# penn-pal-lab/robot_aware_control

Measured on AMD Instinct MI355X. Metric: SVG train frames/sec + CEM candidate-rollouts/sec, 64x64, higher is better.
Workload: dtype fp32 (conv operands as two fp16 parts = 22 significant bits, fp32 accumulate; see fp32_exact)

## Files before the change

### robot_aware_control_amd/csrc/rac_split16.hip

```cpp
#include <math.h>
#include <stdlib.h>

#include <type_traits>

#include "rac_common.h"

namespace rac {

typedef _Float16 f16x8 __attribute__((ext_vector_type(8)));
typedef _Float16 f16x4 __attribute__((ext_vector_type(4)));
typedef unsigned int u32x4 __attribute__((ext_vector_type(4)));
typedef unsigned int u32x2 __attribute__((ext_vector_type(2)));
typedef __amdgpu_buffer_rsrc_t rsrc_t;

constexpr unsigned OOB = 0xFFFFFFF0u;
constexpr int SBN = 128, SBK = 32;

__device__ __forceinline__ const void* uniform_ptr(const void* p) {
  unsigned long long v = reinterpret_cast<unsigned long long>(p);
  unsigned lo = __builtin_amdgcn_readfirstlane((unsigned)v);
  unsigned hi = __builtin_amdgcn_readfirstlane((unsigned)(v >> 32));
  return reinterpret_cast<const void*>(((unsigned long long)hi << 32) | lo);
}
__device__ __forceinline__ rsrc_t make_rsrc(const void* p, unsigned bytes) {
// ... 1560 lines not shown
#pragma unroll
          for (int t = 0; t < HB; ++t) read_frag(t, (tap + 1) % 9, cur * abuf);
        }
        __builtin_amdgcn_sched_barrier(0);
#pragma unroll
        for (int t = HB; t < MB; ++t)
#pragma unroll
          for (int nb = 0; nb < NB; ++nb) acc[t][nb] = mma3(fa[t], fb[nb], acc[t][nb]);
      }
    }
    const int img = p.per_image ? cur_t.m0 / p.HW : 0;
    if (RAC_EXP_PERSIST & 2) {
      unsigned mx = 0;
#pragma unroll
      for (int i = 0; i < MB; ++i)
#pragma unroll
        for (int j = 0; j < NB; ++j)
#pragma unroll
          for (int r = 0; r < 4; ++r) mx = max(mx, absbits(acc[i][j][r]));
      if (p.out_amax) amax_commit(mx, p.out_amax + img);
    } else {
      conv16_epilogue(p, acc, cur_t.m0, wm * MB, nmb, n0 + wn * NT * 32, 0, pow2f(-cur_t.ka), pow2f(-kw), pre, nullptr,
                      p.out_amax ? p.out_amax + img : nullptr);
    }
    if (!has_next) break;
    cur ^= 1;
    cur_t = nxt_t;
    bx = next_bx;
  }
}

__global__ __launch_bounds__(256) void absmax_kernel(const float4* x0, long n0v, const float4* x1, long n1v,
                                                     unsigned* amax) {
  __shared__ unsigned sh[4];
  unsigned m = 0;
  const long stride = (long)gridDim.x * blockDim.x;
  for (long i = (long)blockIdx.x * blockDim.x + threadIdx.x; i < n0v + n1v; i += stride) {
    const float4 v = i < n0v ? x0[i] : x1[i - n0v];
    const unsigned a = __builtin_bit_cast(unsigned, v.x) & 0x7FFFFFFFu, b = __builtin_bit_cast(unsigned, v.y) & 0x7FFFFFFFu,
                   c = __builtin_bit_cast(unsigned, v.z) & 0x7FFFFFFFu, d = __builtin_bit_cast(unsigned, v.w) & 0x7FFFFFFFu;
    m = max(m, max(max(a, b), max(c, d)));
  }
#pragma unroll
  for (int o = 32; o > 0; o >>= 1) m = max(m, (unsigned)__shfl_xor((int)m, o));
  if ((threadIdx.x & 63) == 0) sh[threadIdx.x >> 6] = m;
  __syncthreads();
  if (threadIdx.x == 0) {
    m = max(max(sh[0], sh[1]), max(sh[2], sh[3]));
    if (m > __hip_atomic_load(amax, __ATOMIC_RELAXED, __HIP_MEMORY_SCOPE_AGENT)) atomicMax(amax, m);
  }
}

__device__ __forceinline__ void weight_frag16_block(const float* w, const unsigned* w_amax, unsigned short* out, int Cout,
                                                    int Cin, int taps, int transposed, long ps, long block) {
  const int R = transposed ? Cin : Cout, Kc = transposed ? Cout : Cin;
  const int cch = Kc >> 5;
  const long cell = block * 2 + (threadIdx.x >> 7);
  if (cell >= (long)(R >> 5) * cch * taps) return;
  const float s = pow2f(scale_exp(*w_amax));
  const int tap = (int)(cell % taps);
  const int cc = (int)((cell / taps) % cch);
  const int nt = (int)(cell / ((long)taps * cch));
  const int nb = (threadIdx.x >> 6) & 1, lane = threadIdx.x & 63;
  const int r = nt * 32 + nb * 16 + (lane & 15);
  const int k0 = cc * 32 + 8 * (lane >> 4);
  u32x4 lo, hi;
  if (!transposed) {
    const u32x4* src = reinterpret_cast<const u32x4*>(w + ((long)r * taps + tap) * Cin + k0);
    lo = src[0], hi = src[1];
  } else {
    unsigned v[8];
#pragma unroll
    for (int j = 0; j < 8; ++j)
      v[j] = __builtin_bit_cast(unsigned, w[((long)(k0 + j) * taps + (taps - 1 - tap)) * Cin + r]);
    lo = u32x4{v[0], v[1], v[2], v[3]}, hi = u32x4{v[4], v[5], v[6], v[7]};
  }
  u32x4 q[2];
  split8h(lo, hi, s, q);
  const long o = (cell * 2 + nb) * 512 + lane * 8;
  *reinterpret_cast<u32x4*>(out + o) = q[0];
  *reinterpret_cast<u32x4*>(out + ps + o) = q[1];
}

__global__ void weight_frag16_kernel(const float* w, const unsigned* w_amax, unsigned short* out, int Cout, int Cin,
                                     int taps, int transposed, long ps) {
  weight_frag16_block(w, w_amax, out, Cout, Cin, taps, transposed, ps, blockIdx.x);
}

template <typename Job>
__device__ __forceinline__ int job_of_block(const Job* jobs, int n_jobs, long block) {
  int lo = 0, hi = n_jobs - 1;
  while (lo < hi) {
    const int mid = (lo + hi + 1) >> 1;
    if (jobs[mid].block_begin <= block) lo = mid; else hi = mid - 1;
  }
  return lo;
}

__global__ void weight_frag16_multi_kernel(const rac_frag_job* jobs, int n_jobs) {
  const int j = job_of_block(jobs, n_jobs, blockIdx.x);
  const rac_frag_job q = jobs[j];
  weight_frag16_block(q.w, q.w_amax, q.parts, q.Cout, q.Cin, q.ksize * q.ksize, q.transposed, q.part_stride,
                      blockIdx.x - q.block_begin);
}

__global__ __launch_bounds__(256) void absmax_multi_kernel(const rac_absmax_job* jobs, int n_jobs) {
  __shared__ unsigned sh[4];
  const int j = job_of_block(jobs, n_jobs, blockIdx.x);
  const rac_absmax_job q = jobs[j];
  const long nb = (j + 1 < n_jobs ? jobs[j + 1].block_begin : (long)gridDim.x) - q.block_begin;
  const float4* x = reinterpret_cast<const float4*>(q.x);
  const long nv = q.n >> 2;
  unsigned m = 0;
  for (long i = (blockIdx.x - q.block_begin) * 256 + threadIdx.x; i < nv; i += nb * 256) {
    const float4 v = x[i];
    m = max(m, max(max(absbits(v.x), absbits(v.y)), max(absbits(v.z), absbits(v.w))));
  }
#pragma unroll
  for (int o = 32; o > 0; o >>= 1) m = max(m, (unsigned)__shfl_xor((int)m, o));
  if ((threadIdx.x & 63) == 0) sh[threadIdx.x >> 6] = m;
  __syncthreads();
  if (threadIdx.x == 0) {
    m = max(max(sh[0], sh[1]), max(sh[2], sh[3]));
    if (m > __hip_atomic_load(q.amax, __ATOMIC_RELAXED, __HIP_MEMORY_SCOPE_AGENT)) atomicMax(q.amax, m);
  }
}


__global__ __launch_bounds__(256) void adam_frag_multi_kernel(const rac_adam_frag_job* jobs, int n_jobs, long total_blocks,
                                                              float b1, float b2, float eps, float step_size,
                                                              float inv_sqrt_bc2) {
  __shared__ float tile[2][32][33];
  __shared__ unsigned mx_sh[4];
  for (long blk = blockIdx.x; blk < total_blocks; blk += gridDim.x) {
  const int j = job_of_block(jobs, n_jobs, (int)blk);
  const rac_adam_frag_job q = jobs[j];
  const int taps = q.ksize * q.ksize, cch = q.Cin >> 5;
  const int half = threadIdx.x >> 7;
  const long cell = (blk - q.block_begin) * 2 + half;
  const bool active = cell < (long)(q.Cout >> 5) * cch * taps;
  const int tap = (int)(cell % taps);
  const int cc = (int)((cell / taps) % cch);
  const int nt = (int)(cell / ((long)taps * cch));
  const int nb = (threadIdx.x >> 6) & 1, lane = threadIdx.x & 63;
  const int rl = nb * 16 + (lane & 15), kl = 8 * (lane >> 4);
  const float s = pow2f(scale_exp(*q.scale_slot));
  unsigned mx = 0;
  if (active) {
    const long off = ((long)(nt * 32 + rl) * taps + tap) * q.Cin + cc * 32 + kl;
    f32x4 P[2], G[2], M[2], V[2];
#pragma unroll
    for (int h = 0; h < 2; ++h) {
      P[h] = *reinterpret_cast<const f32x4*>(q.p + off + 4 * h);
      G[h] = *reinterpret_cast<const f32x4*>(q.g + off + 4 * h);
      M[h] = *reinterpret_cast<const f32x4*>(q.m + off + 4 * h);
      V[h] = *reinterpret_cast<const f32x4*>(q.v + off + 4 * h);
#pragma unroll
      for (int e = 0; e < 4; ++e) {
        float pp = P[h][e], mm = M[h][e], vv = V[h][e];
        adam_update(pp, G[h][e], mm, vv, b1, b2, eps, step_size, inv_sqrt_bc2);
        M[h][e] = mm, V[h][e] = vv, P[h][e] = pp;
        mx = max(mx, absbits(pp));
        tile[half][rl][kl + 4 * h + e] = pp;
      }
      *reinterpret_cast<f32x4*>(q.p + off + 4 * h) = P[h];
      *reinterpret_cast<f32x4*>(q.m + off + 4 * h) = M[h];
      *reinterpret_cast<f32x4*>(q.v + off + 4 * h) = V[h];
    }
    if (q.parts_fwd) {
      u32x4 parts[2];
      split8h(__builtin_bit_cast(u32x4, P[0]), __builtin_bit_cast(u32x4, P[1]), s, parts);
      const long o = (cell * 2 + nb) * 512 + lane * 8;
      *reinterpret_cast<u32x4*>(q.parts_fwd + o) = parts[0];
      *reinterpret_cast<u32x4*>(q.parts_fwd + q.part_stride + o) = parts[1];
    }
  }
  __syncthreads();
  if (active && q.parts_t) {
    float v[8];
#pragma unroll
    for (int e = 0; e < 8; ++e) v[e] = tile[half][kl + e][rl];
    u32x4 parts[2];
    split8h(u32x4{__builtin_bit_cast(unsigned, v[0]), __builtin_bit_cast(unsigned, v[1]), __builtin_bit_cast(unsigned, v[2]),
                  __builtin_bit_cast(unsigned, v[3])},
            u32x4{__builtin_bit_cast(unsigned, v[4]), __builtin_bit_cast(unsigned, v[5]), __builtin_bit_cast(unsigned, v[6]),
                  __builtin_bit_cast(unsigned, v[7])}, s, parts);
    const long cell_t = ((long)cc * (q.Cout >> 5) + nt) * taps + (taps - 1 - tap);
    const long o = (cell_t * 2 + nb) * 512 + lane * 8;
    *reinterpret_cast<u32x4*>(q.parts_t + o) = parts[0];
    *reinterpret_cast<u32x4*>(q.parts_t + q.part_stride + o) = parts[1];
  }
#pragma unroll
  for (int o = 32; o > 0; o >>= 1) mx = max(mx, (unsigned)__shfl_xor((int)mx, o));
  if (lane == 0) mx_sh[threadIdx.x >> 6] = mx;
  __syncthreads();
  if (threadIdx.x == 0) {
    mx = max(max(mx_sh[0], mx_sh[1]), max(mx_sh[2], mx_sh[3]));
    if (mx > __hip_atomic_load(q.amax_out, __ATOMIC_RELAXED, __HIP_MEMORY_SCOPE_AGENT)) atomicMax(q.amax_out, mx);
  }
  }
}

__global__ void amax_bound_kernel(unsigned* exact, unsigned* bound, const int* idx, int n, float margin) {
  const int j = blockIdx.x * blockDim.x + threadIdx.x;
  if (j >= n) return;
  const int i = idx[j];
  bound[i] = __builtin_bit_cast(unsigned, __builtin_bit_cast(float, exact[i]) + margin);
  exact[i] = 0;
}


struct Wgrad16P {
  int Bimg, H, W, Cin, Cout, C0, T;
  int R, G;
  int nsplit, accumulate;
  int nseg;
  int x1_skip;
  int presplit;
  const float* dy[RAC_WGRAD_MAX_STEPS];
  const float* x0[RAC_WGRAD_MAX_STEPS];
// ... 566 lines not shown
  u32x4* d0 = reinterpret_cast<u32x4*>(p.parts[t]);
  u32x4* d1 = d0 + p.n8;
  for (long i = (long)blockIdx.x * 256 + threadIdx.x; i < p.n8; i += (long)gridDim.x * 256) {
    u32x4 q[2];
    split8h(src[2 * i], src[2 * i + 1], s, q);
    d0[i] = q[0];
    d1[i] = q[1];
  }
}

__global__ __launch_bounds__(256) void slab_accumulate_many_kernel(const float4* slabs, int n_slabs, long stride4,
                                                                   float4* out, long n4) {
  __shared__ float4 sh[256];
  const int col = threadIdx.x & 15, lane = threadIdx.x >> 4;
  const long i = (long)blockIdx.x * 16 + col;
  float4 a = {0.f, 0.f, 0.f, 0.f};
  if (i < n4)
    for (int s = lane; s < n_slabs; s += 16) {
      const float4 b = slabs[s * stride4 + i];
      a.x += b.x, a.y += b.y, a.z += b.z, a.w += b.w;
    }
  sh[threadIdx.x] = a;
  __syncthreads();
  if (lane == 0 && i < n4) {
    float4 r = out[i];
    for (int k = 0; k < 16; ++k) {
      const float4 b = sh[k * 16 + col];
      r.x += b.x, r.y += b.y, r.z += b.z, r.w += b.w;
    }
    out[i] = r;
  }
}

}

using namespace rac;

extern "C" int rac_absmax(const float* x0, int64_t n0, const float* x1, int64_t n1, uint32_t* amax, void* stream) {
  RAC_REQUIRE(x0 && n0 > 0 && n1 >= 0 && (n1 == 0 || x1) && amax, "rac_absmax: bad args");
  RAC_REQUIRE(n0 % 4 == 0 && n1 % 4 == 0 && aligned16(x0) && (!x1 || aligned16(x1)),
              "rac_absmax: element counts must be multiples of 4, pointers 16-byte aligned");
  long nb = ((n0 + n1) / 4 + 1023) / 1024;
  if (nb > 512) nb = 512;
  hipLaunchKernelGGL(absmax_kernel, dim3((int)nb), dim3(256), 0, reinterpret_cast<hipStream_t>(stream),
                     reinterpret_cast<const float4*>(x0), (long)(n0 / 4), reinterpret_cast<const float4*>(x1),
                     (long)(n1 / 4), amax);
  return check_launch("rac_absmax");
}

extern "C" int rac_weight_frag_split(const float* w, const uint32_t* w_amax, uint16_t* parts, int32_t Cout, int32_t Cin,
                                     int32_t ksize, int32_t transposed, int64_t part_stride, void* stream) {
  RAC_REQUIRE(w && w_amax && parts && Cout > 0 && Cin > 0 && ksize >= 1 && (ksize & 1), "rac_weight_frag_split: bad args");
  RAC_REQUIRE(Cout % 32 == 0 && Cin % 32 == 0, "rac_weight_frag_split: channel counts must be multiples of 32");
  const long n = (long)Cout * Cin * ksize * ksize;
  RAC_REQUIRE(part_stride >= n && part_stride % 8 == 0 && aligned16(w) && aligned16(parts),
              "rac_weight_frag_split: part stride / alignment");
  const long cells = n / 1024;
  hipLaunchKernelGGL(weight_frag16_kernel, dim3((unsigned)((cells + 1) / 2)), dim3(256), 0,
                     reinterpret_cast<hipStream_t>(stream), w, w_amax, parts, Cout, Cin, ksize * ksize, transposed,
                     (long)part_stride);
  return check_launch("rac_weight_frag_split");
}

extern "C" int64_t rac_absmax_blocks(int64_t n) {
  long nb = (n / 4 + 1023) / 1024;
  return nb < 1 ? 1 : (nb > 512 ? 512 : nb);
}

extern "C" int64_t rac_weight_frag_blocks(int32_t Cout, int32_t Cin, int32_t ksize) {
  return ((long)Cout * Cin * ksize * ksize / 1024 + 1) / 2;
}

extern "C" int rac_absmax_multi(const rac_absmax_job* jobs, int32_t n_jobs, int64_t total_blocks, void* stream) {
  RAC_REQUIRE(jobs && n_jobs > 0 && total_blocks >= n_jobs && total_blocks < 0x7FFFFFFFL, "rac_absmax_multi: bad args");
  hipLaunchKernelGGL(absmax_multi_kernel, dim3((unsigned)total_blocks), dim3(256), 0,
                     reinterpret_cast<hipStream_t>(stream), jobs, n_jobs);
  return check_launch("rac_absmax_multi");
}

extern "C" int rac_weight_frag_split_multi(const rac_frag_job* jobs, int32_t n_jobs, int64_t total_blocks, void* stream) {
  RAC_REQUIRE(jobs && n_jobs > 0 && total_blocks >= n_jobs && total_blocks < 0x7FFFFFFFL,
              "rac_weight_frag_split_multi: bad args");
  hipLaunchKernelGGL(weight_frag16_multi_kernel, dim3((unsigned)total_blocks), dim3(256), 0,
                     reinterpret_cast<hipStream_t>(stream), jobs, n_jobs);
  return check_launch("rac_weight_frag_split_multi");
}

extern "C" int rac_adam_frag_multi(const rac_adam_frag_job* jobs, int32_t n_jobs, int64_t total_blocks, float lr, float beta1,
                                   float beta2, float eps, int32_t step, void* stream) {
  RAC_REQUIRE(jobs && n_jobs > 0 && total_blocks >= n_jobs && total_blocks < 0x7FFFFFFFL && step >= 1,
              "rac_adam_frag_multi: bad args");
  const double bc1 = 1.0 - pow((double)beta1, step), bc2 = 1.0 - pow((double)beta2, step);
  hipLaunchKernelGGL(adam_frag_multi_kernel, dim3((unsigned)total_blocks), dim3(256), 0, reinterpret_cast<hipStream_t>(stream),
                     jobs, n_jobs, (long)total_blocks, beta1, beta2, eps, (float)((double)lr / bc1), (float)(1.0 / sqrt(bc2)));
  return check_launch("rac_adam_frag_multi");
}

extern "C" int rac_adam_frag_multi_bounded(const rac_adam_frag_job* jobs, int32_t n_jobs, int64_t total_blocks,
                                           int32_t max_workgroups, float lr, float beta1, float beta2, float eps, int32_t step,
                                           void* stream) {
  RAC_REQUIRE(jobs && n_jobs > 0 && total_blocks > 0 && total_blocks < (1L << 31) && step >= 1 && max_workgroups >= 1,
              "rac_adam_frag_multi_bounded: bad args");
  const double bc1 = 1.0 - pow((double)beta1, step), bc2 = 1.0 - pow((double)beta2, step);
  const long grid = total_blocks < max_workgroups ? total_blocks : max_workgroups;
  hipLaunchKernelGGL(adam_frag_multi_kernel, dim3((unsigned)grid), dim3(256), 0, reinterpret_cast<hipStream_t>(stream), jobs,
                     n_jobs, (long)total_blocks, beta1, beta2, eps, (float)((double)lr / bc1), (float)(1.0 / sqrt(bc2)));
// ... 420 lines not shown
```

### robot_aware_control_amd/ops.py

```python
from __future__ import annotations

import contextlib
import ctypes as C
import functools
import os
import weakref
from typing import Optional, Tuple

import torch

from . import _lib
from ._lib import (AbsmaxJob, AdamFragJob, AdamRange, ConvArgs, FragJob, GradSrc, OptimRange, WgradArgs, call, ptr,
                   stream_ptr)

FWD, DGRAD, WGRAD = 0, 1, 2
ACT_NONE, ACT_LEAKY, ACT_SIGMOID = 0, 1, 2
LOSS_KINDS = {"mse": 0, "l1": 1, "dontcare_mse": 2, "dontcare_l1": 3}
BN_EPS, BN_MOMENTUM = 1e-5, 0.1


def _require_cuda(t: torch.Tensor):
    if not t.is_cuda:
        raise _lib.RacError("robot_aware_control_amd ops run on the GPU only (no CPU fallback); got a CPU tensor")

# ... 2 lines not shown
    co, ci, kh, kw = w.shape
    if w.stride() != (kh * kw * ci, 1, kw * ci, ci):
        raise _lib.RacError(f"conv weight {tuple(w.shape)} must use channels_last memory, strides {w.stride()}")
    return w


_STALE = {}
LAZY_ZERO_GRAD = os.environ.get("RAC_LAZY_ZERO_GRAD", "1") == "1"


def mark_stale(g: torch.Tensor) -> None:
    _STALE[g.data_ptr()] = g


def take_stale(g: torch.Tensor) -> bool:
    return bool(_STALE) and _STALE.pop(g.data_ptr(), None) is not None


def finish_grads() -> None:
    for g in _STALE.values():
        g.zero_()
    _STALE.clear()


def grad_buffer(p: torch.Tensor) -> torch.Tensor:
    if p.grad is None:
        p.grad = torch.zeros_like(p)
    elif _STALE and take_stale(p.grad):
        p.grad.zero_()
    return p.grad


def _cdiv(a, b):
    return (a + b - 1) // b


PARAM_EPOCH = 0


def pad4(c: int) -> int:
    return (-c) % 4


def _derived(weight: torch.Tensor, slot: str, build):
    tag = (weight._version, PARAM_EPOCH, weight.data_ptr())
    hit = getattr(weight, slot, None)
    if hit is not None and hit[0] == tag:
        return hit[1]
    val = build()
    setattr(weight, slot, (tag, val))
    return val


def padded_weight(weight: torch.Tensor, cp: Optional[int] = None) -> torch.Tensor:
    co, ci, k, _ = weight.shape
    cp = ci + pad4(ci) if cp is None else cp

    def build():
        wp = getattr(weight, f"_rac_padbuf{cp}", None)
        if wp is None or wp.device != weight.device:
            wp = torch.empty((co, k, k, cp), device=weight.device, dtype=torch.float32).permute(0, 3, 1, 2)
            setattr(weight, f"_rac_padbuf{cp}", wp)
            wp._rac_pad_source = (weakref.ref(weight), cp)
        call("rac_pad_rows", ptr(weight_mem(weight)), ci, ptr(wp), cp, co * k * k, stream_ptr())
        ent = _WP_ENTRIES.get(id(wp))
        if ent is not None:
            ent.tag = None
        return wp
    return _derived(weight, f"_rac_padded{cp}", build)


def wgrad_padded_acc(dy, x0, weight):
    co, ci, k, _ = weight.shape
    cp = x0.shape[3]
    gp = torch.zeros((co, k, k, cp), device=dy.device, dtype=torch.float32).permute(0, 3, 1, 2)
    B, H, W, Cout = dy.shape
    conv_raw(WGRAD, x0, None, dy, gp, B=B, H=H, W=W, ksize=k, Cin=cp, Cout=Cout, a_split=cp, accumulate=1, split_k=0)
    call("rac_unpad_add", ptr(gp), cp, ptr(weight_mem(grad_buffer(weight))), ci, co * k * k, stream_ptr())


def thin_wgrad_acc(wide, thin, ct: int, weight):
    B, H, W, _ = wide.shape
    n = 64 * 9 * ct
    n_parts = min(512, B * (H // 16) * (W // 16))
    parts = torch.empty((n_parts, n), device=wide.device, dtype=torch.float32)
    sp = stream_ptr()
    call("rac_thin_wgrad", ptr(wide), ptr(thin), thin.shape[3], ct, ptr(parts), n_parts, B, H, W, 64, sp)
    call("rac_slab_accumulate", ptr(parts), n_parts, n, ptr(weight_mem(grad_buffer(weight))), n, sp)


MAX_SPLIT_K = int(os.environ.get("RAC_MAX_SPLIT_K", "8"))


def plan_split_k(M: int, N: int, nchunks: int, tile128_only: bool = False) -> int:
    return _plan_split_k(M, N, nchunks, tile128_only, os.environ.get("RAC_SPLIT"), MAX_SPLIT_K)


@functools.lru_cache(maxsize=None)
def _plan_split_k(M, N, nchunks, tile128_only, forced, max_split):
    if forced:
        return max(1, min(int(forced), nchunks))
    cap = max(1, nchunks // 8)
    if tile128_only:
        t128 = _cdiv(M, 128) * _cdiv(N, 128)
        if t128 >= 384:
            return 1
        best, best_eff = 1, -1.0
        for s in range(1, min(max_split, cap) + 1):
            rounds = t128 * s / 512.0
            eff = (rounds / -(-rounds // 1) if rounds > 1 else rounds) * (1.0 - 0.03 * (s - 1))
            if eff > best_eff + 1e-9:
                best, best_eff = s, eff
        return best
    if N <= 32:
        tiles = _cdiv(M, 128)
        return 1 if tiles >= 384 else max(1, min(8, _cdiv(512, tiles), cap))
    if M >= 128 and N >= 128:
        t128 = _cdiv(M, 128) * _cdiv(N, 128)
        if t128 >= 384:
            return 1
        split = max(1, min(8, _cdiv(512, t128), cap))
        if t128 * split >= 192:
            return split
    tiles = _cdiv(M, 64) * _cdiv(N, 64)
    if tiles >= 384:
        return 1
    return max(1, min(8, _cdiv(512, tiles), cap))


PROFILE = None
SHAPE_LOG = [] if os.environ.get("RAC_SHAPE_LOG") else None
if SHAPE_LOG is not None:
    import atexit
    import json as _json
    atexit.register(lambda: _json.dump(SHAPE_LOG, open(os.environ["RAC_SHAPE_LOG"], "w")))


def _log_shape(family, mode, k, M, N, K, peak):
    SHAPE_LOG.append({"family": family, "mode": ("fwd", "dgrad", "wgrad")[mode], "k": k, "M": M, "N": N, "K": K,
                      "flop": 2.0 * M * N * K, "peak": peak})


def conv_raw(mode: int, a0, a1, w, out0, out1=None, *, B, H, W, ksize, Cin, Cout, act=ACT_NONE, split_k=1,
             slab_stride=0, accumulate=0, a_split=0, o_split=0, bias=None, scale=None, shift=None, stats=None,
             stats_rows=0):
    prof = PROFILE
    if prof is not None and prof["match"] == (mode, ksize, Cin, Cout):
        e0, e1 = torch.cuda.Event(enable_timing=True), torch.cuda.Event(enable_timing=True)
        e0.record()
        _conv_launch(mode, a0, a1, w, out0, out1, B, H, W, ksize, Cin, Cout, act, split_k, slab_stride, accumulate,
                     a_split, o_split, bias, scale, shift, stats, stats_rows)
        e1.record()
        prof["events"].append((e0, e1, B * H * W))
        return
    _conv_launch(mode, a0, a1, w, out0, out1, B, H, W, ksize, Cin, Cout, act, split_k, slab_stride, accumulate,
                 a_split, o_split, bias, scale, shift, stats, stats_rows)


def _conv_launch(mode, a0, a1, w, out0, out1, B, H, W, ksize, Cin, Cout, act, split_k, slab_stride, accumulate,
                 a_split, o_split, bias, scale, shift, stats, stats_rows=0):
    args = ConvArgs(mode=mode, B=B, H=H, W=W, ksize=ksize, Cin=Cin, Cout=Cout, act=act, split_k=split_k,
                    accumulate=accumulate, a_split=a_split, o_split=o_split, slab_stride=slab_stride,
                    a0=ptr(a0), a1=ptr(a1), w=ptr(w), out0=ptr(out0), out1=ptr(out1), bias=ptr(bias),
                    scale=ptr(scale), shift=ptr(shift), stats=ptr(stats), stats_rows=stats_rows)
    if SHAPE_LOG is not None:
        M, N, K = B * H * W, (Cout if mode == FWD else Cin), (Cin if mode == FWD else Cout) * ksize * ksize
        if mode == WGRAD:
            M, N, K = Cout, Cin * ksize * ksize, B * H * W
        _log_shape("igemm", mode, ksize, M, N, K, 157.3)
    call("rac_conv2d", C.byref(args), stream_ptr())


def conv_forward(x0, x1, weight, bias=None, *, act=ACT_NONE, scale=None, shift=None, stats=None,
                 allow_split=True, want_slabs=False, groups=1, frozen=False):
    _require_cuda(x0)
    B, H, W, C0 = x0.shape
    C1 = x1.shape[3] if x1 is not None else 0
    Cout, Cin, k, _ = weight.shape
    assert Cin == C0 + C1, (Cin, C0, C1)
    weight_mem(weight)
    M = B * H * W
    nchunks = k * k * _cdiv(Cin, 32)
    fused = act != ACT_NONE or scale is not None
    split = plan_split_k(M, Cout, nchunks) if (allow_split and not fused and not frozen) else 1
    if want_slabs:
        slabs = torch.empty((split, B, H, W, Cout), device=x0.device, dtype=torch.float32)
        if split == 1:
            conv_raw(FWD, x0, x1, weight, slabs, B=B, H=H, W=W, ksize=k, Cin=Cin, Cout=Cout, a_split=C0)
        else:
            conv_raw(FWD, x0, x1, weight, slabs, B=B, H=H, W=W, ksize=k, Cin=Cin, Cout=Cout, a_split=C0,
                     split_k=split, slab_stride=M * Cout)
        return slabs, split, M * Cout
    out = torch.empty((B, H, W, Cout), device=x0.device, dtype=torch.float32)
    if split == 1:
        conv_raw(FWD, x0, x1, weight, out, B=B, H=H, W=W, ksize=k, Cin=Cin, Cout=Cout, a_split=C0, act=act,
                 bias=bias, scale=scale, shift=shift, stats=stats,
                 stats_rows=(M // groups if (groups > 1 and stats is not None) else 0))
    else:
# ... 135 lines not shown
def broadcast_images(t: torch.Tensor, n: int) -> torch.Tensor:
    out = t.expand(n, *t.shape[1:]).contiguous()
    slot = amax_tag(t)
    if slot is not None:
        if getattr(slot, "_rac_bound1", False):
            tag_amax(out, amax_one(t.device, n))
        elif slot.numel() == 1:
            tag_amax(out, slot.expand(n).contiguous())
    return out


_SPLIT_OK = {}


def split_supported(H: int, W: int, k: int, Cin: int, Cout: int, a_split: int = 0) -> bool:
    key = (H, W, k, Cin, Cout, a_split)
    ok = _SPLIT_OK.get(key)
    if ok is None:
        ok = _SPLIT_OK[key] = bool(_lib.load().rac_conv2d_split_supported(H, W, k, Cin, Cout, a_split))
    return ok


class _WeightParts:
    __slots__ = ("ref", "idx", "slot", "device", "parts", "tag", "exact_ok", "__weakref__")


_WP_ENTRIES = {}
_WP_DEV = {}
_WP_NSLOTS = 1024


def _wp_state(device):
    st = _WP_DEV.get(device)
    if st is None:
        st = _WP_DEV[device] = {"slots": torch.zeros(_WP_NSLOTS, device=device, dtype=torch.int32),
                                "exact": torch.zeros(_WP_NSLOTS, device=device, dtype=torch.int32),
                                "free": list(range(_WP_NSLOTS - 1, -1, -1)), "tables": {}, "adam_plan": None,
                                "optim_plan": None}
    return st


def _wp_drop(key, device, idx, _ref):
    ent = _WP_ENTRIES.get(key)
    if ent is not None and ent.idx == idx and ent.device == device:
        del _WP_ENTRIES[key]
        st = _WP_DEV.get(device)
        if st is not None:
            st["free"].append(idx)


def _wp_tag(weight):
    src = getattr(weight, "_rac_sources", None)
    ver = weight._version if src is None else tuple(t._version for t in src)
    return (ver, PARAM_EPOCH, weight.data_ptr())


def _wp_upload(jobs, device):
    raw = bytes(jobs)
    return torch.frombuffer(bytearray(raw), dtype=torch.uint8).to(device)


ADAM_LATE_WGS = int(os.environ.get("RAC_ADAM_LATE_WGS", "512"))
ADAM_WGS = int(os.environ.get("RAC_ADAM_WGS", "0"))


PARAM_GATE = None


def param_wait(t: torch.Tensor = None) -> None:
    gate = PARAM_GATE
    if gate is None:
        return
    if t is None:
        gate.wait_params()
    elif hasattr(gate, "wait_for"):
        gate.wait_for(t)
    elif not gate.ready(t):
        gate.wait_params()


def _wp_tables(st, items, device):
    lib = _lib.load()
    sig = tuple((w.data_ptr(), ent.idx, tuple(sorted((t, q.data_ptr()) for t, q in ent.parts.items())))
                for ent, w in items)
    tables = st["tables"].get(sig)
    if tables is None:
        if len(st["tables"]) > 8:
            st["tables"].clear()
        ajobs = (AbsmaxJob * len(items))()
        nfrag = sum(len(ent.parts) for ent, _ in items)
        fjobs = (FragJob * nfrag)()
        ab = fb = j = 0
        for i, (ent, w) in enumerate(items):
            wm = weight_mem(w.detach())
            co, ci, k, _ = w.shape
            ajobs[i] = AbsmaxJob(x=ptr(wm), n=wm.numel(), amax=ptr(ent.slot), block_begin=ab)
            ab += lib.rac_absmax_blocks(wm.numel())
            for transposed, parts in sorted(ent.parts.items()):
                fjobs[j] = FragJob(w=ptr(wm), w_amax=ptr(ent.slot), parts=ptr(parts), part_stride=wm.numel(), Cout=co,
                                   Cin=ci, ksize=k, transposed=1 if transposed else 0, block_begin=fb)
                fb += lib.rac_weight_frag_blocks(co, ci, k)
                j += 1
        idx = torch.tensor([ent.idx for ent, _ in items], device=device, dtype=torch.long)
        tables = st["tables"][sig] = (_wp_upload(ajobs, device), len(items), ab, _wp_upload(fjobs, device), nfrag, fb, idx)
    return tables


def _wp_refresh(device):
    st = _wp_state(device)
    stale, n_live = [], 0
    gate = PARAM_GATE
    for ent in list(_WP_ENTRIES.values()):
        if ent.device != device:
            continue
        w = ent.ref()
        if w is None:
            continue
        src = getattr(w, "_rac_pad_source", None)
        if gate is not None:
            base = src[0]() if src is not None else w
            if base is not None and not gate.ready(base):
                continue
        if src is not None:
            param = src[0]()
            if param is None:
                continue
            padded_weight(param, src[1])
        n_live += 1
        if ent.tag != _wp_tag(w):
            stale.append((ent, w))
    if not stale:
        return
    sp = stream_ptr()
    if len(stale) <= 2:
        for ent, w in stale:
            ent.slot.zero_()
            wm = weight_mem(w.detach())
            co, ci, k, _ = w.shape
            call("rac_absmax", ptr(wm), wm.numel(), None, 0, ptr(ent.slot), sp)
            for transposed, parts in ent.parts.items():
                call("rac_weight_frag_split", ptr(wm), ptr(ent.slot), ptr(parts), co, ci, k, 1 if transposed else 0,
                     wm.numel(), sp)
            st["exact"][ent.idx:ent.idx + 1].copy_(ent.slot)
            ent.tag, ent.exact_ok = _wp_tag(w), True
        return
    ta, na, ab, tf, nf, fb, idx = _wp_tables(st, stale, device)
    st["slots"].index_fill_(0, idx, 0)
    call("rac_absmax_multi", ptr(ta), na, ab, sp)
    call("rac_weight_frag_split_multi", ptr(tf), nf, fb, sp)
    st["exact"].index_copy_(0, idx, st["slots"].index_select(0, idx))
    for ent, w in stale:
        ent.tag, ent.exact_ok = _wp_tag(w), True


ADAM_FUSED = os.environ.get("RAC_ADAM_FUSED", "1") == "1"
_ADAM_BOUNDS = {}


def adam_step_bound(beta1: float, beta2: float):
    key = (beta1, beta2)
    if key not in _ADAM_BOUNDS:
        r = beta1 * beta1 / beta2
        if not (0.0 <= beta1 < 1.0 and 0.0 < beta2 < 1.0 and r < 1.0):
            _ADAM_BOUNDS[key] = None
        else:
            best, series, b1t, b2t, rk = 0.0, 0.0, 1.0, 1.0, 1.0
            for _ in range(200000):
                series += rk
                rk *= r
                b1t *= beta1
                b2t *= beta2
                best = max(best, (1 - beta1) ** 2 / (1 - b1t) ** 2 * (1 - b2t) / (1 - beta2) * series)
                if rk < 1e-18 and b1t < 1e-18 and b2t < 1e-9:
                    break
            _ADAM_BOUNDS[key] = best ** 0.5
    return _ADAM_BOUNDS[key]


def _wp_covered(flat):
    dev = flat.device
    base, nbytes = flat.data_ptr(), flat.numel() * 4
    covered = []
    for ent in _WP_ENTRIES.values():
        if ent.device != dev:
            continue
        w = ent.ref()
        if w is None or getattr(w, "_rac_pad_source", None) is not None:
            continue
        off = w.data_ptr() - base
        co, ci, k, _ = w.shape
        if not (0 <= off < nbytes and off % 16 == 0 and w.stride() == (k * k * ci, 1, k * ci, ci)):
            continue
        if ent.tag != _wp_tag(w) or not ent.exact_ok:
            return None
        covered.append((off // 4, ent, w))
    covered.sort(key=lambda c: c[0])
    return covered


def fused_adam_step(flat, grad, m, v, lr, beta1, beta2, eps, step, late=None):
    global PARAM_EPOCH
    if not ADAM_FUSED:
        return False
    bound = adam_step_bound(beta1, beta2)
    if bound is None:
        return False
    dev = flat.device
    st = _wp_state(dev)
    base = flat.data_ptr()
    covered = _wp_covered(flat)
    if not covered:
        return False
    late_sets = [] if late is None else (list(late[1]) if isinstance(late[1], (list, tuple)) else [late[1]])

    def late_group(off, w):
        if late is None or off < late[0]:
            return -1
        for gi, ptrs in enumerate(late_sets):
            if w.data_ptr() in ptrs:
                return gi
        return -1
    is_late = lambda off, w: late_group(off, w) >= 0
    sig = (base, grad.data_ptr(), m.data_ptr(), v.data_ptr(),
           None if late is None else (late[0], tuple(tuple(sorted(ps)) for ps in late_sets)),
           tuple((off, ent.idx, tuple(sorted((t, q.data_ptr()) for t, q in ent.parts.items()))) for off, ent, _ in covered))
    plan = st["adam_plan"]
    if plan is not None and plan["sig"] == sig and plan.get("unsupported"):
        return False
    if plan is None or plan["sig"] != sig:
        lib = _lib.load()
        jobs = (AdamFragJob * len(covered))()
        groups = [late_group(off, w) for off, _, w in covered]
        n_early = sum(1 for gi in groups if gi < 0)
        n_in = [sum(1 for gi in groups if gi == k) for k in range(len(late_sets))]
        first = [n_early + sum(n_in[:k]) for k in range(len(late_sets))]
        slot_of, taken = {}, [0] * len(late_sets)
        ne = 0
        for j, gi in enumerate(groups):
            if gi >= 0:
                slot_of[j], taken[gi] = first[gi] + taken[gi], taken[gi] + 1
            else:
                slot_of[j], ne = ne, ne + 1
        ranges, blocks, pos = [], 0, 0
        late_blocks = [0] * len(late_sets)
        late_spans = [[] for _ in late_sets]
        for i, (off, ent, w) in enumerate(covered):
            co, ci, k, _ = w.shape
            n = w.numel()
            if off % 4 or n % 4 or off < pos or flat.numel() % 4:
                st["adam_plan"] = {"sig": sig, "unsupported": True}
                return False
            if off > pos:
                ranges.append((pos // 4, (off - pos) // 4))
            pos = off + n
            gi = groups[i]
            lt = gi >= 0
            jobs[slot_of[i]] = AdamFragJob(p=base + 4 * off, g=grad.data_ptr() + 4 * off, m=m.data_ptr() + 4 * off,
                                           v=v.data_ptr() + 4 * off, scale_slot=ptr(ent.slot),
                                           amax_out=ptr(st["exact"][ent.idx:ent.idx + 1]), parts_fwd=ptr(ent.parts.get(False)),
                                           parts_t=ptr(ent.parts.get(True)), part_stride=n, Cout=co, Cin=ci, ksize=k, reserved=0,
                                           block_begin=late_blocks[gi] if lt else blocks)
            if lt:
                late_blocks[gi] += lib.rac_weight_frag_blocks(co, ci, k)
                late_spans[gi].append((off, n))
            else:
                blocks += lib.rac_weight_frag_blocks(co, ci, k)
        if pos < flat.numel():
            ranges.append((pos // 4, (flat.numel() - pos + 3) // 4))
        rjobs = (AdamRange * max(1, len(ranges)))()
        rblocks = 0
        for i, (b4, n4) in enumerate(ranges):
            rjobs[i] = AdamRange(begin4=b4, n4=n4, block_begin=rblocks)
            rblocks += _cdiv(n4, 1024)
        plan = st["adam_plan"] = {
            "sig": sig, "jobs": _wp_upload(jobs, dev), "n_jobs": len(covered), "blocks": blocks,
            "n_early": n_early, "late_blocks": late_blocks, "late_spans": late_spans, "late_first": first, "late_n": n_in,
            "ranges": _wp_upload(rjobs, dev), "n_ranges": len(ranges), "rblocks": rblocks,
            "idx": torch.tensor([ent.idx for _, ent, _ in covered], device=dev, dtype=torch.int32)}
    sp = stream_ptr()
    call("rac_amax_bound", ptr(st["exact"]), ptr(st["slots"]), ptr(plan["idx"]), plan["n_jobs"],
         float(lr) * bound * 1.01, sp)
    n_early, n_late = plan["n_early"], plan["n_jobs"] - plan["n_early"]
    if n_early and ADAM_WGS:
        call("rac_adam_frag_multi_bounded", ptr(plan["jobs"]), n_early, plan["blocks"], ADAM_WGS, float(lr), float(beta1),
             float(beta2), float(eps), int(step), sp)
    elif n_early:
        call("rac_adam_frag_multi", ptr(plan["jobs"]), n_early, plan["blocks"], float(lr), float(beta1), float(beta2),
             float(eps), int(step), sp)
    if plan["n_ranges"]:
        call("rac_adam_ranges", ptr(flat), ptr(grad), ptr(m), ptr(v), ptr(plan["ranges"]), plan["n_ranges"],
             plan["rblocks"], float(lr), float(beta1), float(beta2), float(eps), int(step), sp)
    done = []
    if n_late:
        main = torch.cuda.current_stream()
        side = _side_stream("adam", dev)
        ready = torch.cuda.Event()
        ready.record(main)
        side.wait_event(ready)
        with torch.cuda.stream(side):
            for gi, n_g in enumerate(plan["late_n"]):
                if not n_g:
                    continue
                call("rac_adam_frag_multi_bounded", ptr(plan["jobs"]) + plan["late_first"][gi] * C.sizeof(AdamFragJob), n_g,
                     plan["late_blocks"][gi], ADAM_LATE_WGS, float(lr), float(beta1), float(beta2), float(eps), int(step),
                     stream_ptr())
                ev = torch.cuda.Event()
                ev.record(side)
                done.append((ev, list(plan["late_spans"][gi])))
    PARAM_EPOCH += 1
    for _, ent, w in covered:
        ent.tag = _wp_tag(w)
    return done if done else True


def fused_optim_step(rule, flat, grad, state0, state1, lr, momentum=0.0, gain=1.0, alpha=0.0, eps=0.0, flags=0):
    global PARAM_EPOCH
    dev = flat.device
    st = _wp_state(dev)
    base = flat.data_ptr()
    covered = _wp_covered(flat)
    if not covered:
        return False
    sig = (base, grad.data_ptr(), ptr(state0), ptr(state1),
           tuple((off, ent.idx, tuple(sorted((t, q.data_ptr()) for t, q in ent.parts.items()))) for off, ent, _ in covered))
    plan = st["optim_plan"]
    if plan is not None and plan["sig"] == sig and plan.get("unsupported"):
        return False
    if plan is None or plan["sig"] != sig:
        ranges, pos = [], 0
        for off, ent, w in covered:
            n = w.numel()
            if off % 4 or n % 4 or off < pos or off + n > flat.numel() or flat.numel() % 4:
                st["optim_plan"] = {"sig": sig, "unsupported": True}
                return False
            if off > pos:
                ranges.append((pos // 4, (off - pos) // 4, None))
            ranges.append((off // 4, n // 4, ptr(ent.slot)))
            pos = off + n
        if pos < flat.numel():
            ranges.append((pos // 4, (flat.numel() - pos) // 4, None))
        rjobs = (OptimRange * len(ranges))()
        rblocks = 0
        for i, (b4, n4, slot) in enumerate(ranges):
            rjobs[i] = OptimRange(begin4=b4, n4=n4, block_begin=rblocks, amax=slot)
            rblocks += _cdiv(n4, 1024)
        _, _, _, tf, nf, fb, idx = _wp_tables(st, [(ent, w) for _, ent, w in covered], dev)
        plan = st["optim_plan"] = {"sig": sig, "ranges": _wp_upload(rjobs, dev), "n_ranges": len(ranges), "rblocks": rblocks,
                                   "frag": tf, "n_frag": nf, "frag_blocks": fb, "idx": idx}
    sp = stream_ptr()
    idx = plan["idx"]
    st["slots"].index_fill_(0, idx, 0)
    call("rac_optim_ranges", ptr(flat), ptr(grad), ptr(state0), ptr(state1), ptr(plan["ranges"]), plan["n_ranges"],
         plan["rblocks"], int(rule), int(flags), float(lr), float(momentum), float(gain), float(alpha), float(eps), sp)
    call("rac_weight_frag_split_multi", ptr(plan["frag"]), plan["n_frag"], plan["frag_blocks"], sp)
    st["exact"].index_copy_(0, idx, st["slots"].index_select(0, idx))
    PARAM_EPOCH += 1
    for _, ent, w in covered:
        ent.tag = _wp_tag(w)
    return True


def weight_parts(weight: torch.Tensor, transposed: bool = False):
    key = id(weight)
    ent = _WP_ENTRIES.get(key)
    if ent is None or ent.ref() is not weight or ent.device != weight.device:
        st = _wp_state(weight.device)
        if not st["free"]:
            raise _lib.RacError("too many conv weights registered for the split-precision pipe")
        co, ci, k, _ = weight.shape
        if co % 32 or ci % 32:
            raise _lib.RacError(f"split-precision weight {tuple(weight.shape)}: channel counts must be multiples of 32")
        ent = _WeightParts()
        ent.idx = st["free"].pop()
        ent.device, ent.parts, ent.tag, ent.exact_ok = weight.device, {}, None, False
        ent.slot = st["slots"][ent.idx:ent.idx + 1]
        ent.ref = weakref.ref(weight, functools.partial(_wp_drop, key, weight.device, ent.idx))
        _WP_ENTRIES[key] = ent
    if transposed not in ent.parts:
        parts = torch.empty((2, weight.numel()), device=weight.device, dtype=torch.float16)
        parts._rac_transposed = transposed
        ent.parts[transposed] = parts
        ent.tag = None
    if ent.tag != _wp_tag(weight):
        gate = PARAM_GATE
        if gate is not None:
            src = getattr(weight, "_rac_pad_source", None)
            base = src[0]() if src is not None else weight
            if base is not None and not gate.ready(base):
                gate.wait_params()
        _wp_refresh(weight.device)
    return ent.parts[transposed], ent.slot


_CONV_ARGS = {}


def _split_launch(x0, x1, a0, a1, pw, wslot, out, *, B, H, W, k, Cin, Cout, C0, act=ACT_NONE, bias=None, scale=None,
                  shift=None, stats=None, split_k=1, slab_stride=0, stats_rows=0, out_amax=None, w_cin=0, a0_up=0,
                  per_image=False, pool=None):
    key = (B, H, W, k, Cin, Cout, act, split_k, C0, slab_stride, stats_rows, a0_up, per_image)
    args = _CONV_ARGS.get(key)
    if args is None:
        args = _CONV_ARGS[key] = ConvArgs(mode=FWD, B=B, H=H, W=W, ksize=k, Cin=Cin, Cout=Cout, act=act, split_k=split_k,
                                          accumulate=0, a_split=C0, o_split=0, slab_stride=slab_stride, stats_rows=stats_rows,
                                          a0_up=a0_up, amax_per_image=1 if per_image else 0)
    args.a0, args.a1, args.w, args.out0 = ptr(x0), ptr(x1), ptr(pw), ptr(out)
    args.out1 = None if isinstance(pool, str) else ptr(pool)
    args.bias, args.scale, args.shift, args.stats = ptr(bias), ptr(scale), ptr(shift), ptr(stats)
    if isinstance(pool, str):
        return bool(_lib.load().rac_conv2d_fwd_split_pool_ok(C.byref(args), w_cin))
# ... 2036 lines not shown
```

Before: 4298.

## Fuse channel padding into weight fragment split and Adam update for padded convs

Weights whose Cin is not a multiple of 32 used to be copied into a padded buffer (rac_pad_rows) before being split into fp16 fragment parts, and so were excluded from the fused Adam+fragment path. The fragment and Adam-frag kernels now read the unpadded stored weight directly, with a stored-Cin field and zero-filled out-of-range channels. This lets padded weights take part in the fused optimizer step. The padded buffer is now materialized lazily only when a non-WGRAD conv actually needs raw padded values. This adds scalar, non-vectorized loads on the padded path and more complex tag/cache bookkeeping.

```diff
diff --git a/robot_aware_control_amd/csrc/rac_split16.hip b/robot_aware_control_amd/csrc/rac_split16.hip
--- a/robot_aware_control_amd/csrc/rac_split16.hip
+++ b/robot_aware_control_amd/csrc/rac_split16.hip
@@ -1636,7 +1636,9 @@
 }
 
 __device__ __forceinline__ void weight_frag16_block(const float* w, const unsigned* w_amax, unsigned short* out, int Cout,
-                                                    int Cin, int taps, int transposed, long ps, long block) {
+                                                    int Cin, int taps, int tflags, long ps, long block) {
+  const int transposed = tflags & 1;
+  const int Cs = (tflags >> 1) ? (tflags >> 1) : Cin;
   const int R = transposed ? Cin : Cout, Kc = transposed ? Cout : Cin;
   const int cch = Kc >> 5;
   const long cell = block * 2 + (threadIdx.x >> 7);
@@ -1649,14 +1651,20 @@
   const int r = nt * 32 + nb * 16 + (lane & 15);
   const int k0 = cc * 32 + 8 * (lane >> 4);
   u32x4 lo, hi;
-  if (!transposed) {
+  if (!transposed && Cs == Cin) {
     const u32x4* src = reinterpret_cast<const u32x4*>(w + ((long)r * taps + tap) * Cin + k0);
     lo = src[0], hi = src[1];
   } else {
     unsigned v[8];
-#pragma unroll
-    for (int j = 0; j < 8; ++j)
-      v[j] = __builtin_bit_cast(unsigned, w[((long)(k0 + j) * taps + (taps - 1 - tap)) * Cin + r]);
+    if (!transposed) {
+      const float* row = w + ((long)r * taps + tap) * Cs;
+#pragma unroll
+      for (int j = 0; j < 8; ++j) v[j] = k0 + j < Cs ? __builtin_bit_cast(unsigned, row[k0 + j]) : 0u;
+    } else {
+#pragma unroll
+      for (int j = 0; j < 8; ++j)
+        v[j] = r < Cs ? __builtin_bit_cast(unsigned, w[((long)(k0 + j) * taps + (taps - 1 - tap)) * Cs + r]) : 0u;
+    }
     lo = u32x4{v[0], v[1], v[2], v[3]}, hi = u32x4{v[4], v[5], v[6], v[7]};
   }
   u32x4 q[2];
@@ -1719,7 +1727,7 @@
   for (long blk = blockIdx.x; blk < total_blocks; blk += gridDim.x) {
   const int j = job_of_block(jobs, n_jobs, (int)blk);
   const rac_adam_frag_job q = jobs[j];
-  const int taps = q.ksize * q.ksize, cch = q.Cin >> 5;
+  const int taps = q.ksize * q.ksize, cch = (q.reserved ? q.reserved : q.Cin) >> 5;
   const int half = threadIdx.x >> 7;
   const long cell = (blk - q.block_begin) * 2 + half;
   const bool active = cell < (long)(q.Cout >> 5) * cch * taps;
@@ -1733,6 +1741,24 @@
   if (active) {
     const long off = ((long)(nt * 32 + rl) * taps + tap) * q.Cin + cc * 32 + kl;
     f32x4 P[2], G[2], M[2], V[2];
+    if (q.reserved) {
+#pragma unroll
+      for (int h = 0; h < 2; ++h)
+#pragma unroll
+        for (int e = 0; e < 4; ++e) {
+          float pp = 0.f;
+          if (cc * 32 + kl + 4 * h + e < q.Cin) {
+            const long i = off + 4 * h + e;
+            float mm = q.m[i], vv = q.v[i];
+            pp = q.p[i];
+            adam_update(pp, q.g[i], mm, vv, b1, b2, eps, step_size, inv_sqrt_bc2);
+            q.p[i] = pp, q.m[i] = mm, q.v[i] = vv;
+            mx = max(mx, absbits(pp));
+          }
+          P[h][e] = pp;
+          tile[half][rl][kl + 4 * h + e] = pp;
+        }
+    } else {
 #pragma unroll
     for (int h = 0; h < 2; ++h) {
       P[h] = *reinterpret_cast<const f32x4*>(q.p + off + 4 * h);
@@ -1750,6 +1776,7 @@
       *reinterpret_cast<f32x4*>(q.p + off + 4 * h) = P[h];
       *reinterpret_cast<f32x4*>(q.m + off + 4 * h) = M[h];
       *reinterpret_cast<f32x4*>(q.v + off + 4 * h) = V[h];
+    }
     }
     if (q.parts_fwd) {
       u32x4 parts[2];
@@ -2422,6 +2449,7 @@
                                      int32_t ksize, int32_t transposed, int64_t part_stride, void* stream) {
   RAC_REQUIRE(w && w_amax && parts && Cout > 0 && Cin > 0 && ksize >= 1 && (ksize & 1), "rac_weight_frag_split: bad args");
   RAC_REQUIRE(Cout % 32 == 0 && Cin % 32 == 0, "rac_weight_frag_split: channel counts must be multiples of 32");
+  RAC_REQUIRE(transposed >= 0 && (transposed >> 1) <= Cin, "rac_weight_frag_split: stored Cin above the parts' Cin");
   const long n = (long)Cout * Cin * ksize * ksize;
   RAC_REQUIRE(part_stride >= n && part_stride % 8 == 0 && aligned16(w) && aligned16(parts),
               "rac_weight_frag_split: part stride / alignment");
diff --git a/robot_aware_control_amd/ops.py b/robot_aware_control_amd/ops.py
--- a/robot_aware_control_amd/ops.py
+++ b/robot_aware_control_amd/ops.py
@@ -78,9 +78,13 @@
     return val
 
 
+FUSED_PADDED_PARTS = os.environ.get("RAC_FUSED_PADDED_PARTS", "1") == "1"
+
+
 def padded_weight(weight: torch.Tensor, cp: Optional[int] = None) -> torch.Tensor:
     co, ci, k, _ = weight.shape
     cp = ci + pad4(ci) if cp is None else cp
+    lazy = FUSED_PADDED_PARTS
 
     def build():
         wp = getattr(weight, f"_rac_padbuf{cp}", None)
@@ -88,11 +92,30 @@
             wp = torch.empty((co, k, k, cp), device=weight.device, dtype=torch.float32).permute(0, 3, 1, 2)
             setattr(weight, f"_rac_padbuf{cp}", wp)
             wp._rac_pad_source = (weakref.ref(weight), cp)
+        if lazy:
+            return wp
         call("rac_pad_rows", ptr(weight_mem(weight)), ci, ptr(wp), cp, co * k * k, stream_ptr())
         ent = _WP_ENTRIES.get(id(wp))
         if ent is not None:
             ent.tag = None
         return wp
+    if lazy:
+        return build()
+    return _derived(weight, f"_rac_padded{cp}", build)
+
+
+def padded_values(w: torch.Tensor) -> torch.Tensor:
+    src = getattr(w, "_rac_pad_source", None)
+    if src is None or not FUSED_PADDED_PARTS:
+        return w
+    weight, cp = src[0](), src[1]
+    if weight is None:
+        return w
+    co, ci, k, _ = weight.shape
+
+    def build():
+        call("rac_pad_rows", ptr(weight_mem(weight)), ci, ptr(w), cp, co * k * k, stream_ptr())
+        return w
     return _derived(weight, f"_rac_padded{cp}", build)
 
 
@@ -170,6 +193,8 @@
 def conv_raw(mode: int, a0, a1, w, out0, out1=None, *, B, H, W, ksize, Cin, Cout, act=ACT_NONE, split_k=1,
              slab_stride=0, accumulate=0, a_split=0, o_split=0, bias=None, scale=None, shift=None, stats=None,
              stats_rows=0):
+    if mode != WGRAD:
+        w = padded_values(w)
     prof = PROFILE
     if prof is not None and prof["match"] == (mode, ksize, Cin, Cout):
         e0, e1 = torch.cuda.Event(enable_timing=True), torch.cuda.Event(enable_timing=True)
@@ -411,7 +436,20 @@
 def _wp_tag(weight):
     src = getattr(weight, "_rac_sources", None)
     ver = weight._version if src is None else tuple(t._version for t in src)
+    if FUSED_PADDED_PARTS:
+        pad = getattr(weight, "_rac_pad_source", None)
+        base = pad[0]() if pad is not None else None
+        if base is not None:
+            return (base._version, PARAM_EPOCH, weight.data_ptr(), base.data_ptr())
     return (ver, PARAM_EPOCH, weight.data_ptr())
+
+
+def _wp_store(w):
+    pad = getattr(w, "_rac_pad_source", None)
+    base = pad[0]() if (pad is not None and FUSED_PADDED_PARTS) else None
+    if base is None:
+        return weight_mem(w.detach()), 0
+    return weight_mem(base.detach()), base.shape[1] << 1
 
 
 def _wp_upload(jobs, device):
@@ -440,8 +478,8 @@
 
 def _wp_tables(st, items, device):
     lib = _lib.load()
-    sig = tuple((w.data_ptr(), ent.idx, tuple(sorted((t, q.data_ptr()) for t, q in ent.parts.items())))
-                for ent, w in items)
+    sig = tuple((w.data_ptr(), _wp_store(w)[0].data_ptr(), ent.idx,
+                 tuple(sorted((t, q.data_ptr()) for t, q in ent.parts.items()))) for ent, w in items)
     tables = st["tables"].get(sig)
     if tables is None:
         if len(st["tables"]) > 8:
@@ -451,13 +489,13 @@
         fjobs = (FragJob * nfrag)()
         ab = fb = j = 0
         for i, (ent, w) in enumerate(items):
-            wm = weight_mem(w.detach())
+            wm, stored = _wp_store(w)
             co, ci, k, _ = w.shape
             ajobs[i] = AbsmaxJob(x=ptr(wm), n=wm.numel(), amax=ptr(ent.slot), block_begin=ab)
             ab += lib.rac_absmax_blocks(wm.numel())
             for transposed, parts in sorted(ent.parts.items()):
-                fjobs[j] = FragJob(w=ptr(wm), w_amax=ptr(ent.slot), parts=ptr(parts), part_stride=wm.numel(), Cout=co,
-                                   Cin=ci, ksize=k, transposed=1 if transposed else 0, block_begin=fb)
+                fjobs[j] = FragJob(w=ptr(wm), w_amax=ptr(ent.slot), parts=ptr(parts), part_stride=w.numel(), Cout=co,
+                                   Cin=ci, ksize=k, transposed=(1 if transposed else 0) | stored, block_begin=fb)
                 fb += lib.rac_weight_frag_blocks(co, ci, k)
                 j += 1
         idx = torch.tensor([ent.idx for ent, _ in items], device=device, dtype=torch.long)
@@ -484,7 +522,8 @@
             param = src[0]()
             if param is None:
                 continue
-            padded_weight(param, src[1])
+            if not FUSED_PADDED_PARTS:
+                padded_weight(param, src[1])
         n_live += 1
         if ent.tag != _wp_tag(w):
             stale.append((ent, w))
@@ -494,12 +533,12 @@
     if len(stale) <= 2:
         for ent, w in stale:
             ent.slot.zero_()
-            wm = weight_mem(w.detach())
+            wm, stored = _wp_store(w)
             co, ci, k, _ = w.shape
             call("rac_absmax", ptr(wm), wm.numel(), None, 0, ptr(ent.slot), sp)
             for transposed, parts in ent.parts.items():
-                call("rac_weight_frag_split", ptr(wm), ptr(ent.slot), ptr(parts), co, ci, k, 1 if transposed else 0,
-                     wm.numel(), sp)
+                call("rac_weight_frag_split", ptr(wm), ptr(ent.slot), ptr(parts), co, ci, k,
+                     (1 if transposed else 0) | stored, w.numel(), sp)
             st["exact"][ent.idx:ent.idx + 1].copy_(ent.slot)
             ent.tag, ent.exact_ok = _wp_tag(w), True
         return
@@ -539,20 +578,27 @@
 def _wp_covered(flat):
     dev = flat.device
     base, nbytes = flat.data_ptr(), flat.numel() * 4
-    covered = []
+    covered, padded_seen = [], set()
     for ent in _WP_ENTRIES.values():
         if ent.device != dev:
             continue
         w = ent.ref()
-        if w is None or getattr(w, "_rac_pad_source", None) is not None:
+        if w is None:
             continue
-        off = w.data_ptr() - base
-        co, ci, k, _ = w.shape
-        if not (0 <= off < nbytes and off % 16 == 0 and w.stride() == (k * k * ci, 1, k * ci, ci)):
+        s, pad = w, getattr(w, "_rac_pad_source", None)
+        if pad is not None:
+            s = pad[0]() if FUSED_PADDED_PARTS else None
+            if s is None or s.data_ptr() in padded_seen:
+                continue
+        off = s.data_ptr() - base
+        co, ci, k, _ = s.shape
+        if not (0 <= off < nbytes and off % 16 == 0 and s.stride() == (k * k * ci, 1, k * ci, ci)):
             continue
+        if pad is not None:
+            padded_seen.add(s.data_ptr())
         if ent.tag != _wp_tag(w) or not ent.exact_ok:
             return None
-        covered.append((off // 4, ent, w))
+        covered.append((off // 4, ent, w, s))
     covered.sort(key=lambda c: c[0])
     return covered
 
@@ -582,14 +628,14 @@
     is_late = lambda off, w: late_group(off, w) >= 0
     sig = (base, grad.data_ptr(), m.data_ptr(), v.data_ptr(),
            None if late is None else (late[0], tuple(tuple(sorted(ps)) for ps in late_sets)),
-           tuple((off, ent.idx, tuple(sorted((t, q.data_ptr()) for t, q in ent.parts.items()))) for off, ent, _ in covered))
+           tuple((off, ent.idx, tuple(sorted((t, q.data_ptr()) for t, q in ent.parts.items()))) for off, ent, _, _ in covered))
     plan = st["adam_plan"]
     if plan is not None and plan["sig"] == sig and plan.get("unsupported"):
         return False
     if plan is None or plan["sig"] != sig:
         lib = _lib.load()
         jobs = (AdamFragJob * len(covered))()
-        groups = [late_group(off, w) for off, _, w in covered]
+        groups = [late_group(off, s) for off, _, _, s in covered]
         n_early = sum(1 for gi in groups if gi < 0)
         n_in = [sum(1 for gi in groups if gi == k) for k in range(len(late_sets))]
         first = [n_early + sum(n_in[:k]) for k in range(len(late_sets))]
@@ -603,9 +649,9 @@
         ranges, blocks, pos = [], 0, 0
         late_blocks = [0] * len(late_sets)
         late_spans = [[] for _ in late_sets]
-        for i, (off, ent, w) in enumerate(covered):
-            co, ci, k, _ = w.shape
-            n = w.numel()
+        for i, (off, ent, w, s) in enumerate(covered):
+            co, ci, k, _ = s.shape
+            n, cp = s.numel(), w.shape[1]
             if off % 4 or n % 4 or off < pos or flat.numel() % 4:
                 st["adam_plan"] = {"sig": sig, "unsupported": True}
                 return False
@@ -617,13 +663,14 @@
             jobs[slot_of[i]] = AdamFragJob(p=base + 4 * off, g=grad.data_ptr() + 4 * off, m=m.data_ptr() + 4 * off,
                                            v=v.data_ptr() + 4 * off, scale_slot=ptr(ent.slot),
                                            amax_out=ptr(st["exact"][ent.idx:ent.idx + 1]), parts_fwd=ptr(ent.parts.get(False)),
-                                           parts_t=ptr(ent.parts.get(True)), part_stride=n, Cout=co, Cin=ci, ksize=k, reserved=0,
+                                           parts_t=ptr(ent.parts.get(True)), part_stride=w.numel(), Cout=co, Cin=ci, ksize=k,
+                                           reserved=cp if cp != ci else 0,
                                            block_begin=late_blocks[gi] if lt else blocks)
             if lt:
-                late_blocks[gi] += lib.rac_weight_frag_blocks(co, ci, k)
+                late_blocks[gi] += lib.rac_weight_frag_blocks(co, cp, k)
                 late_spans[gi].append((off, n))
             else:
-                blocks += lib.rac_weight_frag_blocks(co, ci, k)
+                blocks += lib.rac_weight_frag_blocks(co, cp, k)
         if pos < flat.numel():
             ranges.append((pos // 4, (flat.numel() - pos + 3) // 4))
         rjobs = (AdamRange * max(1, len(ranges)))()
@@ -635,7 +682,7 @@
             "sig": sig, "jobs": _wp_upload(jobs, dev), "n_jobs": len(covered), "blocks": blocks,
             "n_early": n_early, "late_blocks": late_blocks, "late_spans": late_spans, "late_first": first, "late_n": n_in,
             "ranges": _wp_upload(rjobs, dev), "n_ranges": len(ranges), "rblocks": rblocks,
-            "idx": torch.tensor([ent.idx for _, ent, _ in covered], device=dev, dtype=torch.int32)}
+            "idx": torch.tensor([ent.idx for _, ent, _, _ in covered], device=dev, dtype=torch.int32)}
     sp = stream_ptr()
     call("rac_amax_bound", ptr(st["exact"]), ptr(st["slots"]), ptr(plan["idx"]), plan["n_jobs"],
          float(lr) * bound * 1.01, sp)
@@ -667,7 +714,7 @@
                 ev.record(side)
                 done.append((ev, list(plan["late_spans"][gi])))
     PARAM_EPOCH += 1
-    for _, ent, w in covered:
+    for _, ent, w, _ in covered:
         ent.tag = _wp_tag(w)
     return done if done else True
 
@@ -681,14 +728,14 @@
     if not covered:
         return False
     sig = (base, grad.data_ptr(), ptr(state0), ptr(state1),
-           tuple((off, ent.idx, tuple(sorted((t, q.data_ptr()) for t, q in ent.parts.items()))) for off, ent, _ in covered))
+           tuple((off, ent.idx, tuple(sorted((t, q.data_ptr()) for t, q in ent.parts.items()))) for off, ent, _, _ in covered))
     plan = st["optim_plan"]
     if plan is not None and plan["sig"] == sig and plan.get("unsupported"):
         return False
     if plan is None or plan["sig"] != sig:
         ranges, pos = [], 0
-        for off, ent, w in covered:
-            n = w.numel()
+        for off, ent, _, s in covered:
+            n = s.numel()
             if off % 4 or n % 4 or off < pos or off + n > flat.numel() or flat.numel() % 4:
                 st["optim_plan"] = {"sig": sig, "unsupported": True}
                 return False
@@ -703,7 +750,7 @@
         for i, (b4, n4, slot) in enumerate(ranges):
             rjobs[i] = OptimRange(begin4=b4, n4=n4, block_begin=rblocks, amax=slot)
             rblocks += _cdiv(n4, 1024)
-        _, _, _, tf, nf, fb, idx = _wp_tables(st, [(ent, w) for _, ent, w in covered], dev)
+        _, _, _, tf, nf, fb, idx = _wp_tables(st, [(ent, w) for _, ent, w, _ in covered], dev)
         plan = st["optim_plan"] = {"sig": sig, "ranges": _wp_upload(rjobs, dev), "n_ranges": len(ranges), "rblocks": rblocks,
                                    "frag": tf, "n_frag": nf, "frag_blocks": fb, "idx": idx}
     sp = stream_ptr()
@@ -714,7 +761,7 @@
     call("rac_weight_frag_split_multi", ptr(plan["frag"]), plan["n_frag"], plan["frag_blocks"], sp)
     st["exact"].index_copy_(0, idx, st["slots"].index_select(0, idx))
     PARAM_EPOCH += 1
-    for _, ent, w in covered:
+    for _, ent, w, _ in covered:
         ent.tag = _wp_tag(w)
     return True
 
```

Result: no change. 4279 (-0.4%).
